# zju3dv/pvnet

Measured on NVIDIA H100. Metric: images/sec (480x640, K=9) backbone+vote, higher is better.
Workload: dtype tf32 (fp32 storage, fp32 accumulate; vote fp32/fp64)

## Files before the change

### include/pvnet_b200.h

```cpp
#ifndef PVNET_B200_H_
#define PVNET_B200_H_

#include <stddef.h>
#include <stdint.h>

#ifdef __cplusplus
extern "C" {
#endif

#if defined(__GNUC__)
#define PVNET_API __attribute__((visibility("default")))
#else
#define PVNET_API
#endif

typedef void *pvnet_stream_t;

enum {
    PVNET_OK = 0,
    PVNET_E_INVALID = -1,
    PVNET_E_WORKSPACE = -2,
    PVNET_E_CUDA = -3,
    PVNET_E_STATE = -4
};
// ... 171 lines not shown
    int32_t *counts;
    double *sil_obj;
    int32_t *pair_idx;
    double *normal_eq;
} pvnet_refine_trace_t;
PVNET_API int pvnet_refine_workspace_bytes(int b, int h, int w, int max_points, size_t *bytes);
PVNET_API int pvnet_refine_poses(const uint8_t *mask, const double *poses_in, const float *K, int k_per_image,
                                 const float *verts, const int32_t *faces, int nv, int nf, int b, int h, int w,
                                 float near_clip, float far_clip, int rounds, float gate, int max_points,
                                 double *poses_out, int32_t *info, double *dist, const pvnet_refine_trace_t *trace,
                                 void *workspace, size_t workspace_bytes, pvnet_stream_t stream);

PVNET_API int pvnet_refine_poses_keypoints(const uint8_t *mask, const double *poses_in, const float *K, int k_per_image,
                                           const float *verts, const int32_t *faces, int nv, int nf, int b, int h,
                                           int w, float near_clip, float far_clip, int rounds, float gate,
                                           int max_points, const float *keypoints, const float *points_3d,
                                           const float *weights_2d, int nk, double keypoint_weight, double *poses_out,
                                           int32_t *info, double *dist, double *cost,
                                           const pvnet_refine_trace_t *trace, double *keypoint_eq, void *workspace,
                                           size_t workspace_bytes, pvnet_stream_t stream);

typedef struct {
    int32_t *pair_idx;
    int32_t *counts;
    double *X;
    double *Y;
    double *n;
    double *normal_eq;
} pvnet_refine_depth_trace_t;
PVNET_API int pvnet_refine_depth_workspace_bytes(int b, int h, int w, int max_points, size_t *bytes);
PVNET_API int pvnet_refine_poses_depth(const uint8_t *mask, const void *depth, int depth_is_u16, float depth_scale,
                                       const double *poses_in, const float *K, int k_per_image, const float *verts,
                                       const int32_t *faces, int nv, int nf, int b, int h, int w, float near_clip,
                                       float far_clip, int rounds, double gate, int max_points, double *poses_out,
                                       int32_t *info, double *dist, const pvnet_refine_depth_trace_t *trace,
                                       void *workspace, size_t workspace_bytes, pvnet_stream_t stream);

PVNET_API int pvnet_generate_hypothesis_vanishing_point(const float *direct, const float *coords, const int32_t *idxs,
                                                        float *hypo, int tn, int vn, int hn, pvnet_stream_t stream);
PVNET_API int pvnet_voting_for_hypothesis_vanishing_point(const float *direct, const float *coords, const float *hypo,
                                                          uint8_t *inliers, int32_t *counts, int tn, int vn, int hn,
                                                          float inlier_thresh, pvnet_stream_t stream);

PVNET_API long long pvnet_launch_count(void);
PVNET_API void pvnet_launch_count_reset(void);


PVNET_API int pvnet_conv2d_nhwc(const float *in, int in_cs, int in_co, int Cin,
                                const float *w_packed, const float *bias,
                                const float *res, int res_cs, int res_co,
                                float *out, int out_cs, int out_co, int Cout,
                                int b, int H, int W, int ksize, int stride, int dilation,
                                int act, int round_out, pvnet_stream_t stream);

PVNET_API int pvnet_conv2d_nhwc_wgrad_workspace_bytes(int Cin, int Cout, int b, int H, int W, int ksize,
                                                      size_t *bytes);
PVNET_API int pvnet_conv2d_nhwc_wgrad(const float *in, int in_cs, int in_co, int Cin,
                                      const float *dout, int dout_cs, int dout_co, int Cout, float *dw,
                                      int b, int H, int W, int ksize, int dilation,
                                      void *workspace, size_t workspace_bytes, pvnet_stream_t stream);
PVNET_API int pvnet_zero_insert2x_nhwc(const float *in, int in_cs, int in_co, int C, float *out, int out_cs,
                                       int out_co, int b, int H, int W, pvnet_stream_t stream);

PVNET_API int pvnet_upsample2x_nhwc(const float *in, int C, float *out, int out_cs, int out_co, int b, int h, int w,
                                    pvnet_stream_t stream);
PVNET_API int pvnet_upsample2x_backward_nhwc(const float *dout, int dout_cs, int dout_co, int C, float *din, int b,
                                             int h, int w, pvnet_stream_t stream);

typedef struct pvnet_batchnorm {
    const float *weight;
    const float *bias;
    float *running_mean;
    float *running_var;
    int batch_stats;
    double factor;
    double eps;
    double *saved;
    float *coef;
} pvnet_batchnorm_t;
PVNET_API int pvnet_batchnorm_workspace_bytes(int form, int C, long long npix, size_t *bytes);
PVNET_API int pvnet_batchnorm_act_forward(int form, int act, const float *x, const float *z, long long npix, int C,
                                          const pvnet_batchnorm_t *bn, const pvnet_batchnorm_t *bn_z, float *y,
                                          void *workspace, size_t workspace_bytes, pvnet_stream_t stream);
PVNET_API int pvnet_batchnorm_act_backward(int form, int act, const float *dy, const float *x, const float *z,
                                           long long npix, int C, const pvnet_batchnorm_t *bn,
                                           const pvnet_batchnorm_t *bn_z, float *dx, float *dz, float *dweight,
                                           float *dbias, float *dweight_z, float *dbias_z, void *workspace,
                                           size_t workspace_bytes, pvnet_stream_t stream);

PVNET_API int pvnet_stem_s2d_nhwc(const void *image, int image_is_u8, const float *mean3, const float *std3,
                                  const float *w_s2d, const float *bias, float *s2d, float *out, float *img, int img_cs,
                                  int img_co, int b, int H, int W, pvnet_stream_t stream);
PVNET_API int pvnet_stem_s2d_half_nhwc(const void *image, int image_is_u8, const float *mean3, const float *std3,
                                       const float *w_s2d, const float *bias, float *s2d, float *out, float *img,
                                       int img_cs, int img_co, int b, int H, int W, pvnet_stream_t stream);
PVNET_API int pvnet_stem_s2d_wgrad_workspace_bytes(int b, int H, int W, size_t *bytes);
PVNET_API int pvnet_stem_s2d_wgrad(const float *s2d, const float *dout, float *dw, int b, int H, int W,
                                   void *workspace, size_t workspace_bytes, pvnet_stream_t stream);
PVNET_API int pvnet_maxpool3x3s2_nhwc(const float *in, float *out, uint8_t *code, int b, int H, int W, int C,
                                      pvnet_stream_t stream);
PVNET_API int pvnet_maxpool3x3s2_backward_nhwc(const float *dout, const uint8_t *code, float *din, int b, int H, int W,
                                               int C, pvnet_stream_t stream);
PVNET_API int pvnet_head1x1_nchw(const float *y, const float *w, const float *bias, float *out, int b, int H, int W,
                                 int Cin, int Cout, pvnet_stream_t stream);
PVNET_API int pvnet_head1x1_backward_workspace_bytes(int b, int H, int W, int Cin, int Cout, size_t *bytes);
PVNET_API int pvnet_head1x1_backward(const float *dout, const float *y, const float *w, float *dy, float *dw,
// ... 67 lines not shown
```

### pvnet_b200/_native.py

```python
from __future__ import annotations

import ctypes
import os
import threading

_HERE = os.path.dirname(os.path.abspath(__file__))
LIB_PATH = os.path.join(_HERE, "_lib", "libpvnet_b200.so")

_lock = threading.Lock()
_lib = None

c_void_p = ctypes.c_void_p
c_int = ctypes.c_int
c_float = ctypes.c_float
c_size_t = ctypes.c_size_t
c_int64_p = ctypes.POINTER(ctypes.c_int64)


class BatchNormParams(ctypes.Structure):
    _fields_ = [("weight", c_void_p), ("bias", c_void_p), ("running_mean", c_void_p), ("running_var", c_void_p),
                ("batch_stats", c_int), ("factor", ctypes.c_double), ("eps", ctypes.c_double),
                ("saved", c_void_p), ("coef", c_void_p)]


# ... 97 lines not shown
    "pvnet_refine_depth_workspace_bytes": (c_int, [c_int, c_int, c_int, c_int, ctypes.POINTER(c_size_t)]),
    "pvnet_refine_poses_depth": (c_int, [c_void_p, c_void_p, c_int, c_float, c_void_p, c_void_p, c_int, c_void_p,
                                         c_void_p, c_int, c_int, c_int, c_int, c_int, c_float, c_float, c_int,
                                         ctypes.c_double, c_int, c_void_p, c_void_p, c_void_p,
                                         ctypes.POINTER(RefineDepthTrace), c_void_p, c_size_t, c_void_p]),
    "pvnet_generate_hypothesis":(c_int, [c_void_p, c_void_p, c_void_p, c_void_p, c_int, c_int, c_int, c_void_p]),
    "pvnet_voting_for_hypothesis": (c_int, [c_void_p, c_void_p, c_void_p, c_void_p, c_int, c_int, c_int, c_float,
                                            c_void_p]),
    "pvnet_generate_hypothesis_vanishing_point": (c_int, [c_void_p, c_void_p, c_void_p, c_void_p, c_int, c_int, c_int,
                                                          c_void_p]),
    "pvnet_voting_for_hypothesis_vanishing_point": (c_int, [c_void_p, c_void_p, c_void_p, c_void_p, c_void_p, c_int, c_int,
                                                            c_int, c_float, c_void_p]),
    "pvnet_vote_counts": (c_int, [c_void_p, c_void_p, c_void_p, c_void_p, c_int, c_int, c_int, c_float, c_void_p]),
    "pvnet_conv2d_nhwc": (c_int, [c_void_p, c_int, c_int, c_int, c_void_p, c_void_p, c_void_p, c_int, c_int,
                                  c_void_p, c_int, c_int, c_int, c_int, c_int, c_int, c_int, c_int, c_int,
                                  c_int, c_int, c_void_p]),
    "pvnet_conv2d_nhwc_wgrad_workspace_bytes": (c_int, [c_int, c_int, c_int, c_int, c_int, c_int,
                                                        ctypes.POINTER(c_size_t)]),
    "pvnet_conv2d_nhwc_wgrad": (c_int, [c_void_p, c_int, c_int, c_int, c_void_p, c_int, c_int, c_int, c_void_p,
                                        c_int, c_int, c_int, c_int, c_int, c_void_p, c_size_t, c_void_p]),
    "pvnet_zero_insert2x_nhwc": (c_int, [c_void_p, c_int, c_int, c_int, c_void_p, c_int, c_int, c_int, c_int, c_int,
                                         c_void_p]),
    "pvnet_upsample2x_nhwc": (c_int, [c_void_p, c_int, c_void_p, c_int, c_int, c_int, c_int, c_int, c_void_p]),
    "pvnet_upsample2x_backward_nhwc": (c_int, [c_void_p, c_int, c_int, c_int, c_void_p, c_int, c_int, c_int, c_void_p]),
    "pvnet_batchnorm_workspace_bytes": (c_int, [c_int, c_int, ctypes.c_longlong, ctypes.POINTER(c_size_t)]),
    "pvnet_batchnorm_act_forward": (c_int, [c_int, c_int, c_void_p, c_void_p, ctypes.c_longlong, c_int, c_bn_p, c_bn_p,
                                            c_void_p, c_void_p, c_size_t, c_void_p]),
    "pvnet_batchnorm_act_backward": (c_int, [c_int, c_int, c_void_p, c_void_p, c_void_p, ctypes.c_longlong, c_int,
                                             c_bn_p, c_bn_p, c_void_p, c_void_p, c_void_p, c_void_p, c_void_p, c_void_p,
                                             c_void_p, c_size_t, c_void_p]),
    "pvnet_stem_s2d_nhwc": (c_int, [c_void_p, c_int, ctypes.POINTER(c_float), ctypes.POINTER(c_float), c_void_p,
                                    c_void_p, c_void_p, c_void_p, c_void_p, c_int, c_int, c_int, c_int, c_int,
                                    c_void_p]),
    "pvnet_stem_s2d_half_nhwc": (c_int, [c_void_p, c_int, ctypes.POINTER(c_float), ctypes.POINTER(c_float), c_void_p,
                                         c_void_p, c_void_p, c_void_p, c_void_p, c_int, c_int, c_int, c_int, c_int,
                                         c_void_p]),
    "pvnet_stem_s2d_wgrad_workspace_bytes": (c_int, [c_int, c_int, c_int, ctypes.POINTER(c_size_t)]),
    "pvnet_stem_s2d_wgrad": (c_int, [c_void_p, c_void_p, c_void_p, c_int, c_int, c_int, c_void_p, c_size_t, c_void_p]),
    "pvnet_maxpool3x3s2_nhwc": (c_int, [c_void_p, c_void_p, c_void_p, c_int, c_int, c_int, c_int, c_void_p]),
    "pvnet_maxpool3x3s2_backward_nhwc": (c_int, [c_void_p, c_void_p, c_void_p, c_int, c_int, c_int, c_int, c_void_p]),
    "pvnet_head1x1_nchw": (c_int, [c_void_p, c_void_p, c_void_p, c_void_p, c_int, c_int, c_int, c_int, c_int,
                                   c_void_p]),
    "pvnet_head1x1_backward_workspace_bytes": (c_int, [c_int, c_int, c_int, c_int, c_int, ctypes.POINTER(c_size_t)]),
    "pvnet_head1x1_backward": (c_int, [c_void_p, c_void_p, c_void_p, c_void_p, c_void_p, c_void_p, c_int, c_int,
                                       c_int, c_int, c_int, c_void_p, c_size_t, c_void_p]),
    "pvnet_head3x3_nchw": (c_int, [c_void_p, c_void_p, c_void_p, c_void_p, c_int, c_int, c_int, c_int, c_void_p]),
    "pvnet_head3x3_backward_workspace_bytes": (c_int, [c_int, c_int, c_int, c_int, ctypes.POINTER(c_size_t)]),
    "pvnet_head3x3_backward": (c_int, [c_void_p, c_void_p, c_void_p, c_void_p, c_void_p, c_void_p, c_int, c_int,
                                       c_int, c_int, c_void_p, c_size_t, c_void_p]),
    "pvnet_adam_step": (c_int, [ctypes.POINTER(AdamTensor), c_int, ctypes.c_double, ctypes.c_double, ctypes.c_double,
                                ctypes.c_double, ctypes.c_double, ctypes.c_int64, c_void_p]),
    "pvnet_adam_chunk_tensors": (c_int, []),
    "pvnet_conv_set_mode": (c_int, [c_int]),
    "pvnet_backbone_create": (c_int, [c_int, c_int, c_int, c_int, c_int, c_int, c_int, ctypes.POINTER(c_void_p)]),
    "pvnet_backbone_create_trunk": (c_int, [c_int, ctypes.POINTER(c_int), c_int, c_int, c_int, c_int, c_int, c_int,
                                            c_int, ctypes.POINTER(c_void_p)]),
    "pvnet_backbone_create_trunk_2o": (c_int, [c_int, ctypes.POINTER(c_int), c_int, c_int, c_int, c_int, c_int,
                                               c_int, ctypes.POINTER(c_void_p)]),
    "pvnet_backbone_create_detector": (c_int, [c_int, ctypes.POINTER(c_int), c_int, ctypes.POINTER(c_void_p)]),
    "pvnet_backbone_output_scale": (c_int, [c_void_p]),
    "pvnet_backbone_destroy": (None, [c_void_p]),
    "pvnet_backbone_num_convs": (c_int, []),
    "pvnet_backbone_handle_num_convs": (c_int, [c_void_p]),
    "pvnet_backbone_set_conv": (c_int, [c_void_p, c_int, c_void_p, c_void_p]),
    "pvnet_backbone_set_output_layout": (c_int, [c_void_p, c_int]),
    "pvnet_backbone_workspace_bytes": (c_int, [c_void_p, c_int, c_int, c_int, ctypes.POINTER(c_size_t)]),
    "pvnet_backbone_forward": (c_int, [c_void_p, c_void_p, c_int, c_int, c_int, c_void_p, c_void_p, c_int,
                                       c_void_p, c_size_t, c_void_p]),
    "pvnet_backbone_forward_u8": (c_int, [c_void_p, c_void_p, ctypes.POINTER(c_float), ctypes.POINTER(c_float), c_int, c_int,
                                          c_int, c_void_p, c_void_p, c_int, c_void_p, c_size_t, c_void_p]),
    "pvnet_jpeg_available": (c_int, []),
    "pvnet_jpeg_decoder_create": (c_int, [ctypes.POINTER(c_void_p)]),
    "pvnet_jpeg_decoder_destroy": (None, [c_void_p]),
    "pvnet_jpeg_decode_batch": (c_int, [c_void_p, ctypes.POINTER(ctypes.c_char_p), ctypes.POINTER(c_size_t), c_int, c_int,
                                        c_int, c_void_p, c_void_p]),
    "pvnet_backbone_num_stages": (c_int, []),
    "pvnet_backbone_stage_name": (ctypes.c_char_p, [c_int]),
    "pvnet_backbone_handle_num_stages": (c_int, [c_void_p]),
    "pvnet_backbone_handle_stage_name": (ctypes.c_char_p, [c_void_p, c_int]),
    "pvnet_backbone_run_stage": (c_int, [c_void_p, c_int, c_void_p, c_int, c_int, c_int, c_void_p, c_void_p, c_int,
                                         c_void_p, c_size_t, c_void_p]),
}


def lib():
    global _lib
    if _lib is None:
        with _lock:
            if _lib is None:
                if not os.path.exists(LIB_PATH):
                    raise RuntimeError(
                        f"{LIB_PATH} is missing: build it with `python -m pvnet_b200._build` "
                        "(or __graft_entry__.build()).  pvnet_b200 has no CPU or PyTorch fallback.")
                L = ctypes.CDLL(LIB_PATH)
                for name, (res, args) in SIGNATURES.items():
                    fn = getattr(L, name)
                    fn.restype = res
                    fn.argtypes = args
                _lib = L
    return _lib


def check(status: int, what: str):
    if status != 0:
        msg = lib().pvnet_last_error()
        raise RuntimeError(f"{what} failed (status {status}): {msg.decode() if msg else '?'}")
# ... 9 lines not shown
```

### pvnet_b200/conv.py

```python
from __future__ import annotations

import ctypes

import torch
from torch.autograd.function import once_differentiable

from . import _native

ACT_NONE, ACT_RELU, ACT_LEAKY = 0, 1, 2
MODE_AUTO, MODE_PER_TAP, MODE_COLUMN = 0, 1, 2


def set_mode(mode: int):
    _native.check(_native.lib().pvnet_conv_set_mode(int(mode)), "pvnet_conv_set_mode")


def round_tf32(t: torch.Tensor) -> torch.Tensor:
    i = t.contiguous().view(torch.int32)
    i = (i + 0x1000) & ~0x1FFF
    return i.view(torch.float32)


def fold_bn(weight, bn_weight=None, bn_bias=None, bn_mean=None, bn_var=None, eps=1e-5, conv_bias=None):
    w = weight.detach().to(torch.float64)
    cout = w.shape[0]
    b = torch.zeros(cout, dtype=torch.float64, device=w.device) if conv_bias is None else conv_bias.detach().double()
    if bn_weight is not None:
        scale = bn_weight.detach().double() / torch.sqrt(bn_var.detach().double() + eps)
        w = w * scale[:, None, None, None]
        b = (b - bn_mean.detach().double()) * scale + bn_bias.detach().double()
    return w.float(), b.float()


def cin_padded(cin: int) -> int:
    return 16 if cin == 16 else (cin + 31) // 32 * 32


def pack_weight(w: torch.Tensor, cin_pad: int | None = None, cout_pad: int | None = None, tf32: bool = True):
    cout, cin, kh, kw = w.shape
    cin_pad = cin_padded(cin) if cin_pad is None else cin_pad
    cout_pad = cout if cout_pad is None else cout_pad
    p = torch.zeros(cout_pad, kh * kw, cin_pad, dtype=torch.float32, device=w.device)
    p[:cout, :, :cin] = w.permute(0, 2, 3, 1).reshape(cout, kh * kw, cin)
    return round_tf32(p) if tf32 else p.contiguous()


def pack_stem_s2d(w: torch.Tensor) -> torch.Tensor:
    cout = w.shape[0]
    out = torch.zeros(cout, 4, 4, 16, dtype=torch.float32, device=w.device)
    for ty in range(4):
        for py in range(2):
            kh = 2 * ty + py - 1
            if not 0 <= kh <= 6:
                continue
            for tx in range(4):
                for px in range(2):
                    kw = 2 * tx + px - 1
                    if not 0 <= kw <= 6:
                        continue
                    ch = (py * 2 + px) * 3
                    out[:, ty, tx, ch:ch + 3] = w[:, :, kh, kw]
    return round_tf32(out)


def _p(t):
    return None if t is None else ctypes.c_void_p(t.data_ptr())

# ... 596 lines not shown
```

### pvnet_b200/csrc/conv_tc.cu

```cuda
#include "conv_tc.cuh"
#include "ptx.cuh"

#include <cstdlib>
#include <mutex>
#include <new>

namespace pvnet {

struct ConvGeom {
    int Ho, Wo;
    int tiles_x, tiles_y, total_m_tiles;
    int TH, TW;
    int taps, cin_chunks, cin_pad;
    int Cout, BN;
    int out_cs, out_co;
    int res_cs, res_co;
    int act;
    int round_out;
    signed char tap_map[9];
    short tap_ox[9], tap_oy[9];
    int n_items;
    int stages;
};

struct AMaps {
    CUtensorMap m[4];
};

constexpr int CONV_THREADS = 288;
constexpr int CONV_KC = 32;
constexpr int CONV_A_BYTES = 128 * CONV_KC * 4;
constexpr int CONV_SLAB = 32;
constexpr int CONV_SLAB_BYTES = 128 * CONV_SLAB * 4;
constexpr int CONV_EPI_BAR = 1;

template <int BN>
__global__ void __launch_bounds__(CONV_THREADS, 1)
    k_conv_tap(const __grid_constant__ AMaps amaps, const __grid_constant__ CUtensorMap tmB,
               const __grid_constant__ CUtensorMap tmOut, const __grid_constant__ CUtensorMap tmRes,
               const __grid_constant__ ConvGeom g, const float *__restrict__ bias, const int has_res)
{
    constexpr int B_BYTES = BN * CONV_KC * 4;
    constexpr int STAGE_BYTES = CONV_A_BYTES + B_BYTES;
    constexpr int SLABS = BN / CONV_SLAB;
    const int STAGES = g.stages;
    extern __shared__ uint8_t smem_raw[];
    uint8_t *smem = reinterpret_cast<uint8_t *>((reinterpret_cast<uintptr_t>(smem_raw) + 1023) & ~uintptr_t(1023));
    uint8_t *slab = smem + (size_t)STAGES * STAGE_BYTES;
    uint64_t *full = reinterpret_cast<uint64_t *>(slab + 2 * CONV_SLAB_BYTES);
    uint64_t *empty = full + STAGES;
    uint64_t *res_full = empty + STAGES;
    uint64_t *res_free = res_full + 2;

    const int warp = threadIdx.x >> 5, lane = threadIdx.x & 31;
    const int tiles_per_img = g.tiles_x * g.tiles_y;
    const int n_tiles_n = g.Cout / BN;
    const int nkb = g.taps * g.cin_chunks;
    const int unit = (int)blockIdx.x, nunits = (int)gridDim.x;
    auto item_tile = [&](int item, int &m_tile, int &n0) {
        m_tile = item / n_tiles_n;
        n0 = (item - m_tile * n_tiles_n) * BN;
    };

    if (threadIdx.x == 0) {
        for (int s = 0; s < STAGES; ++s) {
            ptx::mbar_init(&full[s], 1);
            ptx::mbar_init(&empty[s], 8);
        }
        for (int i = 0; i < 2; ++i) {
            ptx::mbar_init(&res_full[i], 1);
            ptx::mbar_init(&res_free[i], 1);
        }
        ptx::fence_barrier_init();
    }
    __syncthreads();

    if (warp == 8) {
        if (lane == 0) {
            int r_item = has_res ? unit : g.n_items, r_slab = 0;
            uint32_t rq = 0;
            auto poll_res = [&]() {
                if (r_item >= g.n_items) return;
                const uint32_t b = rq & 1u;
                if (!ptx::mbar_test_wait(&res_free[b], ((rq >> 1) & 1u) ^ 1u)) return;
                int m_tile, n0;
                item_tile(r_item, m_tile, n0);
                const int img = m_tile / tiles_per_img;
                const int trem = m_tile - img * tiles_per_img;
                const int tyi = trem / g.tiles_x, txi = trem - tyi * g.tiles_x;
                ptx::mbar_arrive_expect_tx(&res_full[b], (uint32_t)CONV_SLAB_BYTES);
                ptx::tma_load_4d(slab + b * CONV_SLAB_BYTES, &tmRes, &res_full[b], n0 + r_slab * CONV_SLAB, txi * g.TW,
                                 tyi * g.TH, img);
                ++rq;
                if (++r_slab == SLABS) {
                    r_slab = 0;
                    r_item += nunits;
                }
            };
            int s = 0;
            uint32_t ph = 0;
            for (int item = unit; item < g.n_items; item += nunits) {
                int m_tile, n0;
                item_tile(item, m_tile, n0);
                const int img = m_tile / tiles_per_img;
                const int trem = m_tile - img * tiles_per_img;
                const int tyi = trem / g.tiles_x, txi = trem - tyi * g.tiles_x;
                const int y0 = tyi * g.TH, x0 = txi * g.TW;
                for (int tap = 0; tap < g.taps; ++tap)
                    for (int cc = 0; cc < g.cin_chunks; ++cc) {
                        poll_res();
                        while (!(has_res ? ptx::mbar_test_wait(&empty[s], ph ^ 1u) : ptx::mbar_try_wait(&empty[s], ph ^ 1u)))
                            poll_res();
                        ptx::mbar_arrive_expect_tx(&full[s], (uint32_t)STAGE_BYTES);
                        uint8_t *sa = smem + (size_t)s * STAGE_BYTES;
                        ptx::tma_load_4d(sa, &amaps.m[g.tap_map[tap]], &full[s], cc * CONV_KC, x0 + g.tap_ox[tap],
                                         y0 + g.tap_oy[tap], img);
                        ptx::tma_load_2d(sa + CONV_A_BYTES, &tmB, &full[s], tap * g.cin_pad + cc * CONV_KC, n0);
                        if (++s == STAGES) {
                            s = 0;
                            ph ^= 1u;
                        }
                    }
            }
            while (r_item < g.n_items) poll_res();
        }
    } else {
        const int wg = warp >> 2, wq = warp & 3;
        const int g8 = lane >> 2, t4 = lane & 3;
        const uint32_t smem_u = ptx::smem_u32(smem);
        int s = 0;
        uint32_t ph = 0, sq = 0;
        for (int item = unit; item < g.n_items; item += nunits) {
            float acc[BN / 2];
#pragma unroll
            for (int i = 0; i < BN / 2; ++i) acc[i] = 0.f;
            int prev = -1;
            for (int kb = 0; kb < nkb; ++kb) {
                ptx::mbar_wait(&full[s], ph);
                const uint32_t sa = smem_u + (uint32_t)s * (uint32_t)STAGE_BYTES;
                const uint64_t adesc = ptx::make_kmajor_desc(sa + (uint32_t)(wg * 64 * 128), 128);
                const uint64_t bdesc = ptx::make_kmajor_desc(sa + (uint32_t)CONV_A_BYTES, 128);
                ptx::wgmma_fence();
#pragma unroll
                for (int k = 0; k < CONV_KC / 8; ++k)
                    ptx::Wgmma<BN>::ss(acc, adesc + (uint64_t)(2 * k), bdesc + (uint64_t)(2 * k), (kb | k) != 0 ? 1u : 0u);
                ptx::wgmma_commit();
                ptx::wgmma_wait<1>();
                ptx::fence_regs(acc);
                if (prev >= 0 && lane == 0) ptx::mbar_arrive(&empty[prev]);
                prev = s;
                if (++s == STAGES) {
                    s = 0;
                    ph ^= 1u;
                }
            }
            ptx::wgmma_wait<0>();
            ptx::fence_regs(acc);
            if (lane == 0) ptx::mbar_arrive(&empty[prev]);

            int m_tile, n0;
            item_tile(item, m_tile, n0);
            const int img = m_tile / tiles_per_img;
            const int trem = m_tile - img * tiles_per_img;
            const int tyi = trem / g.tiles_x, txi = trem - tyi * g.tiles_x;
            const uint32_t row_off = (uint32_t)((wg * 64 + wq * 16 + g8) * 128 + (t4 & 1) * 8);
            const uint32_t swz = (uint32_t)(((t4 >> 1) ^ g8) << 4);
            const uint32_t slab_u = ptx::smem_u32(slab);
#pragma unroll
            for (int j = 0; j < SLABS; ++j, ++sq) {
                const uint32_t b = sq & 1u;
                const uint32_t base = slab_u + b * (uint32_t)CONV_SLAB_BYTES + row_off;
                float2 bv[4];
#pragma unroll
                for (int jj = 0; jj < 4; ++jj)
                    bv[jj] = __ldg(reinterpret_cast<const float2 *>(bias + n0 + CONV_SLAB * j + 8 * jj + 2 * t4));
                if (has_res) ptx::mbar_wait(&res_full[b], (sq >> 1) & 1u);
                else ptx::named_bar_sync(CONV_EPI_BAR, 256);
#pragma unroll
                for (int jj = 0; jj < 4; ++jj)
#pragma unroll
                    for (int h = 0; h < 2; ++h) {
                        const uint32_t addr = base + (uint32_t)(h * 8 * 128) + (swz ^ (uint32_t)(32 * jj));
                        const int a = 4 * (4 * j + jj) + 2 * h;
                        float2 v = make_float2(acc[a] + bv[jj].x, acc[a + 1] + bv[jj].y);
                        if (has_res) {
                            const float2 r = ptx::lds64(addr);
                            v.x += r.x;
                            v.y += r.y;
                        }
                        v.x = epi_act(v.x, g.act, g.round_out);
                        v.y = epi_act(v.y, g.act, g.round_out);
                        ptx::sts64(addr, v);
                    }
                ptx::fence_proxy_async();
                ptx::named_bar_sync(CONV_EPI_BAR, 256);
                if (threadIdx.x == 0) {
                    ptx::tma_store_4d(&tmOut, slab + b * CONV_SLAB_BYTES, n0 + CONV_SLAB * j, txi * g.TW, tyi * g.TH, img);
                    ptx::tma_store_commit();
                    if (j == SLABS - 1) ptx::tma_store_wait_read();
                    else ptx::tma_store_wait_read1();
                    if (has_res) {
                        if (j > 0) ptx::mbar_arrive(&res_free[b ^ 1u]);
                        if (j == SLABS - 1) ptx::mbar_arrive(&res_free[b]);
                    }
                }
                __syncwarp();
            }
        }
        if (threadIdx.x == 0) ptx::tma_store_wait_all();
    }
}

typedef CUresult (*EncodeTiledFn)(CUtensorMap *, CUtensorMapDataType, cuuint32_t, void *, const cuuint64_t *,
                                  const cuuint64_t *, const cuuint32_t *, const cuuint32_t *, CUtensorMapInterleave,
                                  CUtensorMapSwizzle, CUtensorMapL2promotion, CUtensorMapFloatOOBfill);

static EncodeTiledFn encode_fn()
{
    static EncodeTiledFn fn = nullptr;
    static std::once_flag once;
    std::call_once(once, [] {
        void *p = nullptr;
        cudaDriverEntryPointQueryResult q;
        if (cudaGetDriverEntryPoint("cuTensorMapEncodeTiled", &p, cudaEnableDefault, &q) == cudaSuccess &&
            q == cudaDriverEntryPointSuccess)
            fn = reinterpret_cast<EncodeTiledFn>(p);
    });
    return fn;
}

int tma_encode(CUtensorMap *m, const void *base, int rank, const cuuint64_t *dims, const cuuint64_t *strides_bytes,
               const cuuint32_t *box, int swizzle_bytes)
{
    EncodeTiledFn fn = encode_fn();
    if (!fn) {
        set_error("cuTensorMapEncodeTiled entry point unavailable");
        return PVNET_E_CUDA;
    }
    cuuint32_t estr[5] = {1, 1, 1, 1, 1};
    const CUtensorMapSwizzle sw = swizzle_bytes == 128 ? CU_TENSOR_MAP_SWIZZLE_128B
                                  : swizzle_bytes == 64 ? CU_TENSOR_MAP_SWIZZLE_64B
                                                        : CU_TENSOR_MAP_SWIZZLE_32B;
    CUresult r = fn(m, CU_TENSOR_MAP_DATA_TYPE_FLOAT32, (cuuint32_t)rank, const_cast<void *>(base), dims,
                    strides_bytes, box, estr, CU_TENSOR_MAP_INTERLEAVE_NONE, sw, CU_TENSOR_MAP_L2_PROMOTION_L2_128B,
                    CU_TENSOR_MAP_FLOAT_OOB_FILL_NONE);
    if (r == CUDA_ERROR_INVALID_CONTEXT || r == CUDA_ERROR_NOT_INITIALIZED) {
        cudaFree(nullptr);
        r = fn(m, CU_TENSOR_MAP_DATA_TYPE_FLOAT32, (cuuint32_t)rank, const_cast<void *>(base), dims, strides_bytes, box, estr,
               CU_TENSOR_MAP_INTERLEAVE_NONE, sw, CU_TENSOR_MAP_L2_PROMOTION_L2_128B, CU_TENSOR_MAP_FLOAT_OOB_FILL_NONE);
    }
    if (r != CUDA_SUCCESS) {
        set_error("cuTensorMapEncodeTiled failed with CUresult %d (rank %d, dims %llu %llu, box %u %u, swizzle %d)",
                  (int)r, rank, (unsigned long long)dims[0], (unsigned long long)dims[1], box[0], box[1],
                  swizzle_bytes);
        return PVNET_E_CUDA;
    }
    return PVNET_OK;
}

struct ConvPlan {
    AMaps amaps;
    CUtensorMap tmB;
    CUtensorMap tmOut, tmRes;
    ConvGeom g;
    dim3 grid;
    size_t smem;
    const float *bias;
    int has_res;
};

int conv_plan(const ConvDesc &d, ConvPlan *p)
{
    PV_CHECK_ARG(d.in && d.w && d.bias && d.out, "conv: null pointer");
    PV_CHECK_ARG(!d.in2, "conv: a second input source is only supported by the column kernel");
    PV_CHECK_ARG(d.ksize == 1 || d.ksize == 3, "conv: kernel size %d unsupported", d.ksize);
    PV_CHECK_ARG(d.stride == 1 || d.stride == 2, "conv: stride %d unsupported", d.stride);
    PV_CHECK_ARG(d.stride == 1 || (d.dilation == 1 && d.H % 2 == 0 && d.W % 2 == 0),
                 "conv: stride 2 needs dilation 1 and even H,W");
    PV_CHECK_ARG(d.Cout % 32 == 0, "conv: Cout %d must be a multiple of 32", d.Cout);
    PV_CHECK_ARG(d.in_cs % 4 == 0 && d.in_co % 4 == 0 && d.out_cs % 4 == 0 && d.out_co % 4 == 0,
                 "conv: channel strides/offsets must be multiples of 4 floats");
    PV_CHECK_ARG(!d.res || (d.res_cs % 4 == 0 && d.res_co % 4 == 0), "conv: residual stride/offset alignment");
    PV_CHECK_ARG(((uintptr_t)d.in % 16 == 0) && ((uintptr_t)d.w % 16 == 0) && ((uintptr_t)d.out % 16 == 0) &&
                     ((uintptr_t)d.bias % 16 == 0),
                 "conv: pointers must be 16-byte aligned");
    PV_CHECK_ARG(d.Cin % 4 == 0, "conv: Cin %d must be a multiple of 4", d.Cin);
    const int kc = CONV_KC;
    ConvGeom &g = p->g;
    g.Ho = d.H / d.stride;
    g.Wo = d.W / d.stride;
    g.TH = 8;
    g.TW = 16;
    g.tiles_x = (g.Wo + g.TW - 1) / g.TW;
    g.tiles_y = (g.Ho + g.TH - 1) / g.TH;
    g.total_m_tiles = g.tiles_x * g.tiles_y * d.b;
    g.taps = d.ksize * d.ksize;
    g.cin_chunks = (d.Cin + kc - 1) / kc;
    g.cin_pad = g.cin_chunks * kc;
    g.Cout = d.Cout;
    {
        const long long sms = sm_count() > 0 ? sm_count() : 1;
        long long best = -1;
        for (int bn = 256; bn >= 32; bn >>= 1) {
            if (d.Cout % bn) continue;
            const long long items = (long long)g.total_m_tiles * (d.Cout / bn);
            const long long cost = (items + sms - 1) / sms * (CONV_A_BYTES + bn * kc * 4);
            if (best < 0 || cost < best) {
                best = cost;
                g.BN = bn;
            }
        }
    }
    g.out_cs = d.out_cs;
    g.out_co = d.out_co;
    g.res_cs = d.res_cs;
    g.res_co = d.res_co;
    g.act = d.act;
    g.round_out = d.round_out;
    const int pad = d.dilation * (d.ksize - 1) / 2;
    for (int t = 0; t < g.taps; ++t) {
        const int kh = t / d.ksize, kw = t - kh * d.ksize;
        if (d.stride == 1) {
            g.tap_map[t] = 0;
            g.tap_ox[t] = (short)(kw * d.dilation - pad);
            g.tap_oy[t] = (short)(kh * d.dilation - pad);
        } else {
            const int dy = kh - pad, dx = kw - pad;
            const int py = dy & 1, px = dx & 1;
            g.tap_map[t] = (signed char)(py * 2 + px);
            g.tap_oy[t] = (short)((dy - py) / 2);
            g.tap_ox[t] = (short)((dx - px) / 2);
        }
    }
    const int swz = kc * 4;
    const int nplanes = d.stride == 2 ? 4 : 1;
    for (int pl = 0; pl < nplanes; ++pl) {
        const int py = pl >> 1, px = pl & 1;
        const float *base = d.in + d.in_co + ((size_t)py * d.W + px) * d.in_cs;
        cuuint64_t dims[4] = {(cuuint64_t)d.Cin, (cuuint64_t)(d.W / d.stride), (cuuint64_t)(d.H / d.stride),
                              (cuuint64_t)d.b};
        cuuint64_t strides[3] = {(cuuint64_t)d.stride * d.in_cs * 4, (cuuint64_t)d.stride * d.W * d.in_cs * 4,
                                 (cuuint64_t)d.H * d.W * d.in_cs * 4};
        cuuint32_t box[4] = {(cuuint32_t)kc, (cuuint32_t)g.TW, (cuuint32_t)g.TH, 1};
        int rc = tma_encode(&p->amaps.m[pl], base, 4, dims, strides, box, swz);
        if (rc) return rc;
    }
    for (int pl = nplanes; pl < 4; ++pl) p->amaps.m[pl] = p->amaps.m[0];
    {
        cuuint64_t dims[2] = {(cuuint64_t)g.taps * g.cin_pad, (cuuint64_t)d.Cout};
        cuuint64_t strides[1] = {(cuuint64_t)g.taps * g.cin_pad * 4};
        cuuint32_t box[2] = {(cuuint32_t)kc, (cuuint32_t)g.BN};
        int rc = tma_encode(&p->tmB, d.w, 2, dims, strides, box, swz);
        if (rc) return rc;
    }
    {
        cuuint64_t dims[4] = {(cuuint64_t)d.Cout, (cuuint64_t)g.Wo, (cuuint64_t)g.Ho, (cuuint64_t)d.b};
        cuuint32_t box[4] = {(cuuint32_t)CONV_SLAB, (cuuint32_t)g.TW, (cuuint32_t)g.TH, 1};
        cuuint64_t ostr[3] = {(cuuint64_t)d.out_cs * 4, (cuuint64_t)g.Wo * d.out_cs * 4,
                              (cuuint64_t)g.Ho * g.Wo * d.out_cs * 4};
        int rc = tma_encode(&p->tmOut, d.out + d.out_co, 4, dims, ostr, box, CONV_SLAB * 4);
        if (rc) return rc;
        p->tmRes = p->tmOut;
        if (d.res) {
            PV_CHECK_ARG((uintptr_t)d.res % 16 == 0, "conv: pointers must be 16-byte aligned");
            cuuint64_t rstr[3] = {(cuuint64_t)d.res_cs * 4, (cuuint64_t)g.Wo * d.res_cs * 4,
                                  (cuuint64_t)g.Ho * g.Wo * d.res_cs * 4};
            rc = tma_encode(&p->tmRes, d.res + d.res_co, 4, dims, rstr, box, CONV_SLAB * 4);
            if (rc) return rc;
        }
    }
    const size_t stage_b = (size_t)CONV_A_BYTES + (size_t)g.BN * kc * 4;
    int st = (int)((227 * 1024 - 1024 - 256 - 2 * CONV_SLAB_BYTES) / stage_b);
    if (st > 8) st = 8;
    g.stages = st;
    p->smem = 1024 + (size_t)st * stage_b + 2 * CONV_SLAB_BYTES + 256;
    g.n_items = g.total_m_tiles * (d.Cout / g.BN);
    long long grid = (long long)sm_count();
    if (grid > g.n_items) grid = g.n_items;
    p->grid = dim3((unsigned)grid);
    p->bias = d.bias;
    p->has_res = d.res != nullptr;
    return PVNET_OK;
}

template <int BN>
int conv_launch_t(const ConvPlan &p, cudaStream_t s)
{
    const cudaError_t attr_err = ensure_max_smem((const void *)k_conv_tap<BN>, 227 * 1024);
    PV_CUDA(attr_err);
    k_conv_tap<BN><<<p.grid, CONV_THREADS, p.smem, s>>>(p.amaps, p.tmB, p.tmOut, p.tmRes, p.g, p.bias, p.has_res);
    PV_LAUNCHED("k_conv_tap");
    return PVNET_OK;
}

int conv_launch(const ConvPlan &p, cudaStream_t s)
{
    if (p.g.BN == 256) return conv_launch_t<256>(p, s);
    if (p.g.BN == 128) return conv_launch_t<128>(p, s);
    if (p.g.BN == 64) return conv_launch_t<64>(p, s);
    return conv_launch_t<32>(p, s);
}

size_t conv_plan_size() { return sizeof(ConvPlan); }
int conv_plan_at(const ConvDesc &d, void *storage) { return conv_plan(d, new (storage) ConvPlan()); }
int conv_launch_at(const void *storage, cudaStream_t s) { return conv_launch(*static_cast<const ConvPlan *>(storage), s); }

}

extern "C" {

int pvnet_conv2d_nhwc(const float *in, int in_cs, int in_co, int Cin, const float *w_packed, const float *bias,
                      const float *res, int res_cs, int res_co, float *out, int out_cs, int out_co, int Cout, int b,
                      int H, int W, int ksize, int stride, int dilation, int act, int round_out,
                      pvnet_stream_t stream)
{
    pvnet::ConvDesc d{in, in_cs, in_co, Cin, w_packed, bias, res, res_cs, res_co, out, out_cs, out_co, Cout,
                      b, H, W, ksize, stride, dilation, act, round_out};
    const bool col = pvnet::g_conv_mode == 2 || (pvnet::g_conv_mode == 0 && pvnet::conv_col_eligible(d));
    if (col) {
        alignas(64) unsigned char storage[2048];
        static_assert(sizeof(storage) >= 1024, "plan storage");
        if (pvnet::conv_col_plan_size() > sizeof(storage)) {
            pvnet::set_error("column plan larger than its stack storage");
            return PVNET_E_STATE;
        }
        int rc = pvnet::conv_col_plan_at(d, nullptr, storage);
        if (rc) return rc;
        return pvnet::conv_col_launch_at(storage, (cudaStream_t)stream);
    }
    pvnet::ConvPlan plan;
    int rc = pvnet::conv_plan(d, &plan);
    if (rc) return rc;
    return pvnet::conv_launch(plan, (cudaStream_t)stream);
}

}
```

Before: 1720.

## Add cost-model tile scheduler with tail-split launches and multi-image tiles

Replaces the simple BN choice in the tap conv with a cost model that estimates k-block clocks per BN and decides whether to split the work into two launches: a main launch with full waves and a tail launch with a smaller BN that fits in one wave. It also considers a 4x16x2-image tile geometry that changes how many M tiles there are and how they quantize against the SM count. The goal is to cut wave-quantization idle time on the last partial wave of the persistent grid. In exchange it adds an extra launch, and its heuristic constants (feed rate, launch overhead) could choose a worse schedule for some layers. A debug API that exposes the schedule is also added.

```diff
diff --git a/include/pvnet_b200.h b/include/pvnet_b200.h
--- a/include/pvnet_b200.h
+++ b/include/pvnet_b200.h
@@ -247,6 +247,9 @@
                                 float *out, int out_cs, int out_co, int Cout,
                                 int b, int H, int W, int ksize, int stride, int dilation,
                                 int act, int round_out, pvnet_stream_t stream);
+
+PVNET_API int pvnet_conv_tap_schedule(int b, int H, int W, int Cin, int Cout, int ksize, int stride, int sms,
+                                      int *out, int out_len);
 
 PVNET_API int pvnet_conv2d_nhwc_wgrad_workspace_bytes(int Cin, int Cout, int b, int H, int W, int ksize,
                                                       size_t *bytes);
diff --git a/pvnet_b200/_native.py b/pvnet_b200/_native.py
--- a/pvnet_b200/_native.py
+++ b/pvnet_b200/_native.py
@@ -173,6 +173,7 @@
                                 ctypes.c_double, ctypes.c_double, ctypes.c_int64, c_void_p]),
     "pvnet_adam_chunk_tensors": (c_int, []),
     "pvnet_conv_set_mode": (c_int, [c_int]),
+    "pvnet_conv_tap_schedule": (c_int, [c_int, c_int, c_int, c_int, c_int, c_int, c_int, c_int, c_void_p, c_int]),
     "pvnet_backbone_create": (c_int, [c_int, c_int, c_int, c_int, c_int, c_int, c_int, ctypes.POINTER(c_void_p)]),
     "pvnet_backbone_create_trunk": (c_int, [c_int, ctypes.POINTER(c_int), c_int, c_int, c_int, c_int, c_int, c_int,
                                             c_int, ctypes.POINTER(c_void_p)]),
diff --git a/pvnet_b200/conv.py b/pvnet_b200/conv.py
--- a/pvnet_b200/conv.py
+++ b/pvnet_b200/conv.py
@@ -13,6 +13,15 @@
 
 def set_mode(mode: int):
     _native.check(_native.lib().pvnet_conv_set_mode(int(mode)), "pvnet_conv_set_mode")
+
+
+def tap_schedule(b: int, H: int, W: int, cin: int, cout: int, ksize: int, stride: int = 1, sms: int = 132) -> dict:
+    out = (ctypes.c_int * 17)()
+    _native.check(_native.lib().pvnet_conv_tap_schedule(int(b), int(H), int(W), int(cin), int(cout), int(ksize),
+                                                        int(stride), int(sms), out, 17), "pvnet_conv_tap_schedule")
+    v = list(out)
+    launches = [dict(zip(("bn", "m0", "m_tiles", "items", "grid"), v[7 + 5 * i:12 + 5 * i])) for i in range(v[6])]
+    return dict(zip(("th", "tw", "ti", "tiles_x", "tiles_y", "m_tiles"), v[:6]), launches=launches)
 
 
 def round_tf32(t: torch.Tensor) -> torch.Tensor:
diff --git a/pvnet_b200/csrc/conv_tc.cu b/pvnet_b200/csrc/conv_tc.cu
--- a/pvnet_b200/csrc/conv_tc.cu
+++ b/pvnet_b200/csrc/conv_tc.cu
@@ -10,7 +10,8 @@
 struct ConvGeom {
     int Ho, Wo;
     int tiles_x, tiles_y, total_m_tiles;
-    int TH, TW;
+    int TH, TW, TI;
+    int m0;
     int taps, cin_chunks, cin_pad;
     int Cout, BN;
     int out_cs, out_co;
@@ -53,13 +54,22 @@
     uint64_t *res_free = res_full + 2;
 
     const int warp = threadIdx.x >> 5, lane = threadIdx.x & 31;
-    const int tiles_per_img = g.tiles_x * g.tiles_y;
+    const int tiles_per_grp = g.tiles_x * g.tiles_y;
     const int n_tiles_n = g.Cout / BN;
     const int nkb = g.taps * g.cin_chunks;
     const int unit = (int)blockIdx.x, nunits = (int)gridDim.x;
     auto item_tile = [&](int item, int &m_tile, int &n0) {
-        m_tile = item / n_tiles_n;
-        n0 = (item - m_tile * n_tiles_n) * BN;
+        const int mi = item / n_tiles_n;
+        m_tile = g.m0 + mi;
+        n0 = (item - mi * n_tiles_n) * BN;
+    };
+    auto tile_origin = [&](int m_tile, int &x0, int &y0, int &img) {
+        const int grp = m_tile / tiles_per_grp;
+        const int trem = m_tile - grp * tiles_per_grp;
+        const int tyi = trem / g.tiles_x;
+        x0 = (trem - tyi * g.tiles_x) * g.TW;
+        y0 = tyi * g.TH;
+        img = grp * g.TI;
     };
 
     if (threadIdx.x == 0) {
@@ -83,14 +93,11 @@
                 if (r_item >= g.n_items) return;
                 const uint32_t b = rq & 1u;
                 if (!ptx::mbar_test_wait(&res_free[b], ((rq >> 1) & 1u) ^ 1u)) return;
-                int m_tile, n0;
+                int m_tile, n0, x0, y0, img;
                 item_tile(r_item, m_tile, n0);
-                const int img = m_tile / tiles_per_img;
-                const int trem = m_tile - img * tiles_per_img;
-                const int tyi = trem / g.tiles_x, txi = trem - tyi * g.tiles_x;
+                tile_origin(m_tile, x0, y0, img);
                 ptx::mbar_arrive_expect_tx(&res_full[b], (uint32_t)CONV_SLAB_BYTES);
-                ptx::tma_load_4d(slab + b * CONV_SLAB_BYTES, &tmRes, &res_full[b], n0 + r_slab * CONV_SLAB, txi * g.TW,
-                                 tyi * g.TH, img);
+                ptx::tma_load_4d(slab + b * CONV_SLAB_BYTES, &tmRes, &res_full[b], n0 + r_slab * CONV_SLAB, x0, y0, img);
                 ++rq;
                 if (++r_slab == SLABS) {
                     r_slab = 0;
@@ -100,12 +107,9 @@
             int s = 0;
             uint32_t ph = 0;
             for (int item = unit; item < g.n_items; item += nunits) {
-                int m_tile, n0;
+                int m_tile, n0, x0, y0, img;
                 item_tile(item, m_tile, n0);
-                const int img = m_tile / tiles_per_img;
-                const int trem = m_tile - img * tiles_per_img;
-                const int tyi = trem / g.tiles_x, txi = trem - tyi * g.tiles_x;
-                const int y0 = tyi * g.TH, x0 = txi * g.TW;
+                tile_origin(m_tile, x0, y0, img);
                 for (int tap = 0; tap < g.taps; ++tap)
                     for (int cc = 0; cc < g.cin_chunks; ++cc) {
                         poll_res();
@@ -158,11 +162,9 @@
             ptx::fence_regs(acc);
             if (lane == 0) ptx::mbar_arrive(&empty[prev]);
 
-            int m_tile, n0;
+            int m_tile, n0, x0, y0, img;
             item_tile(item, m_tile, n0);
-            const int img = m_tile / tiles_per_img;
-            const int trem = m_tile - img * tiles_per_img;
-            const int tyi = trem / g.tiles_x, txi = trem - tyi * g.tiles_x;
+            tile_origin(m_tile, x0, y0, img);
             const uint32_t row_off = (uint32_t)((wg * 64 + wq * 16 + g8) * 128 + (t4 & 1) * 8);
             const uint32_t swz = (uint32_t)(((t4 >> 1) ^ g8) << 4);
             const uint32_t slab_u = ptx::smem_u32(slab);
@@ -195,7 +197,7 @@
                 ptx::fence_proxy_async();
                 ptx::named_bar_sync(CONV_EPI_BAR, 256);
                 if (threadIdx.x == 0) {
-                    ptx::tma_store_4d(&tmOut, slab + b * CONV_SLAB_BYTES, n0 + CONV_SLAB * j, txi * g.TW, tyi * g.TH, img);
+                    ptx::tma_store_4d(&tmOut, slab + b * CONV_SLAB_BYTES, n0 + CONV_SLAB * j, x0, y0, img);
                     ptx::tma_store_commit();
                     if (j == SLABS - 1) ptx::tma_store_wait_read();
                     else ptx::tma_store_wait_read1();
@@ -258,13 +260,91 @@
     return PVNET_OK;
 }
 
+struct TapLaunch {
+    int bn;
+    int m0, m_tiles;
+    int n_items, grid;
+};
+struct TapSchedule {
+    int TH, TW, TI, tiles_x, tiles_y, total_m_tiles;
+    int nlaunch;
+    TapLaunch l[2];
+};
+
+constexpr long long TAP_RHO = 36;
+constexpr long long TAP_LAUNCH_CLOCKS = 8000;
+
+static long long tap_kblock_clocks(int bn)
+{
+    const long long mma = 1024LL * bn / 256;
+    const long long feed = ((long long)CONV_A_BYTES + (long long)bn * CONV_KC * 4 + TAP_RHO - 1) / TAP_RHO;
+    return mma > feed ? mma : feed;
+}
+
+static long long tap_launches(int Cout, int nkb, int sms, TapSchedule *t)
+{
+    const long long M = t->total_m_tiles, S = sms > 0 ? sms : 1;
+    auto rounds = [&](long long items) { return (items + S - 1) / S; };
+    long long best = -1;
+    for (int bn = 256; bn >= 32; bn >>= 1) {
+        if (Cout % bn) continue;
+        const long long nn = Cout / bn;
+        const long long one = rounds(M * nn) * nkb * tap_kblock_clocks(bn);
+        if (best < 0 || one < best) {
+            best = one;
+            t->nlaunch = 1;
+            t->l[0] = {bn, 0, (int)M, 0, 0};
+        }
+        const long long mm = (M * nn / S) * S / nn;
+        if (mm == 0 || mm == M) continue;
+        int bt = 0;
+        for (int c = 32; c < bn && !bt; c <<= 1)
+            if (Cout % c == 0 && (M - mm) * (Cout / c) <= S) bt = c;
+        if (!bt) continue;
+        const long long two =
+            rounds(mm * nn) * nkb * tap_kblock_clocks(bn) + nkb * tap_kblock_clocks(bt) + TAP_LAUNCH_CLOCKS;
+        if (two < best) {
+            best = two;
+            t->nlaunch = 2;
+            t->l[0] = {bn, 0, (int)mm, 0, 0};
+            t->l[1] = {bt, (int)mm, (int)(M - mm), 0, 0};
+        }
+    }
+    for (int i = 0; i < t->nlaunch; ++i) {
+        TapLaunch &l = t->l[i];
+        l.n_items = l.m_tiles * (Cout / l.bn);
+        l.grid = (int)(S < l.n_items ? S : l.n_items);
+    }
+    return best;
+}
+
+static void tap_schedule(int b, int Ho, int Wo, int Cout, int nkb, int sms, TapSchedule *t)
+{
+    auto geometry = [&](TapSchedule *u, int th, int ti) {
+        u->TW = 16;
+        u->TH = th;
+        u->TI = ti;
+        u->tiles_x = (Wo + u->TW - 1) / u->TW;
+        u->tiles_y = (Ho + u->TH - 1) / u->TH;
+        u->total_m_tiles = u->tiles_x * u->tiles_y * (b / u->TI);
+    };
+    geometry(t, 8, 1);
+    const long long cost = tap_launches(Cout, nkb, sms, t);
+    if (b % 2 == 0 && Ho % 4 == 0 && Wo % 16 == 0) {
+        TapSchedule u{};
+        geometry(&u, 4, 2);
+        if (tap_launches(Cout, nkb, sms, &u) < cost) *t = u;
+    }
+}
+
 struct ConvPlan {
     AMaps amaps;
-    CUtensorMap tmB;
     CUtensorMap tmOut, tmRes;
-    ConvGeom g;
-    dim3 grid;
-    size_t smem;
+    CUtensorMap tmB[2];
+    ConvGeom g[2];
+    dim3 grid[2];
+    size_t smem[2];
+    int nlaunch;
     const float *bias;
     int has_res;
 };
@@ -286,31 +366,21 @@
                  "conv: pointers must be 16-byte aligned");
     PV_CHECK_ARG(d.Cin % 4 == 0, "conv: Cin %d must be a multiple of 4", d.Cin);
     const int kc = CONV_KC;
-    ConvGeom &g = p->g;
+    ConvGeom g{};
     g.Ho = d.H / d.stride;
     g.Wo = d.W / d.stride;
-    g.TH = 8;
-    g.TW = 16;
-    g.tiles_x = (g.Wo + g.TW - 1) / g.TW;
-    g.tiles_y = (g.Ho + g.TH - 1) / g.TH;
-    g.total_m_tiles = g.tiles_x * g.tiles_y * d.b;
     g.taps = d.ksize * d.ksize;
     g.cin_chunks = (d.Cin + kc - 1) / kc;
     g.cin_pad = g.cin_chunks * kc;
+    TapSchedule t;
+    tap_schedule(d.b, g.Ho, g.Wo, d.Cout, g.taps * g.cin_chunks, sm_count(), &t);
+    g.TH = t.TH;
+    g.TW = t.TW;
+    g.TI = t.TI;
+    g.tiles_x = t.tiles_x;
+    g.tiles_y = t.tiles_y;
+    g.total_m_tiles = t.total_m_tiles;
     g.Cout = d.Cout;
-    {
-        const long long sms = sm_count() > 0 ? sm_count() : 1;
-        long long best = -1;
-        for (int bn = 256; bn >= 32; bn >>= 1) {
-            if (d.Cout % bn) continue;
-            const long long items = (long long)g.total_m_tiles * (d.Cout / bn);
-            const long long cost = (items + sms - 1) / sms * (CONV_A_BYTES + bn * kc * 4);
-            if (best < 0 || cost < best) {
-                best = cost;
-                g.BN = bn;
-            }
-        }
-    }
     g.out_cs = d.out_cs;
     g.out_co = d.out_co;
     g.res_cs = d.res_cs;
@@ -318,18 +388,18 @@
     g.act = d.act;
     g.round_out = d.round_out;
     const int pad = d.dilation * (d.ksize - 1) / 2;
-    for (int t = 0; t < g.taps; ++t) {
-        const int kh = t / d.ksize, kw = t - kh * d.ksize;
+    for (int tp = 0; tp < g.taps; ++tp) {
+        const int kh = tp / d.ksize, kw = tp - kh * d.ksize;
         if (d.stride == 1) {
-            g.tap_map[t] = 0;
-            g.tap_ox[t] = (short)(kw * d.dilation - pad);
-            g.tap_oy[t] = (short)(kh * d.dilation - pad);
+            g.tap_map[tp] = 0;
+            g.tap_ox[tp] = (short)(kw * d.dilation - pad);
+            g.tap_oy[tp] = (short)(kh * d.dilation - pad);
         } else {
             const int dy = kh - pad, dx = kw - pad;
             const int py = dy & 1, px = dx & 1;
-            g.tap_map[t] = (signed char)(py * 2 + px);
-            g.tap_oy[t] = (short)((dy - py) / 2);
-            g.tap_ox[t] = (short)((dx - px) / 2);
+            g.tap_map[tp] = (signed char)(py * 2 + px);
+            g.tap_oy[tp] = (short)((dy - py) / 2);
+            g.tap_ox[tp] = (short)((dx - px) / 2);
         }
     }
     const int swz = kc * 4;
@@ -341,21 +411,14 @@
                               (cuuint64_t)d.b};
         cuuint64_t strides[3] = {(cuuint64_t)d.stride * d.in_cs * 4, (cuuint64_t)d.stride * d.W * d.in_cs * 4,
                                  (cuuint64_t)d.H * d.W * d.in_cs * 4};
-        cuuint32_t box[4] = {(cuuint32_t)kc, (cuuint32_t)g.TW, (cuuint32_t)g.TH, 1};
+        cuuint32_t box[4] = {(cuuint32_t)kc, (cuuint32_t)g.TW, (cuuint32_t)g.TH, (cuuint32_t)g.TI};
         int rc = tma_encode(&p->amaps.m[pl], base, 4, dims, strides, box, swz);
         if (rc) return rc;
     }
     for (int pl = nplanes; pl < 4; ++pl) p->amaps.m[pl] = p->amaps.m[0];
     {
-        cuuint64_t dims[2] = {(cuuint64_t)g.taps * g.cin_pad, (cuuint64_t)d.Cout};
-        cuuint64_t strides[1] = {(cuuint64_t)g.taps * g.cin_pad * 4};
-        cuuint32_t box[2] = {(cuuint32_t)kc, (cuuint32_t)g.BN};
-        int rc = tma_encode(&p->tmB, d.w, 2, dims, strides, box, swz);
-        if (rc) return rc;
-    }
-    {
         cuuint64_t dims[4] = {(cuuint64_t)d.Cout, (cuuint64_t)g.Wo, (cuuint64_t)g.Ho, (cuuint64_t)d.b};
-        cuuint32_t box[4] = {(cuuint32_t)CONV_SLAB, (cuuint32_t)g.TW, (cuuint32_t)g.TH, 1};
+        cuuint32_t box[4] = {(cuuint32_t)CONV_SLAB, (cuuint32_t)g.TW, (cuuint32_t)g.TH, (cuuint32_t)g.TI};
         cuuint64_t ostr[3] = {(cuuint64_t)d.out_cs * 4, (cuuint64_t)g.Wo * d.out_cs * 4,
                               (cuuint64_t)g.Ho * g.Wo * d.out_cs * 4};
         int rc = tma_encode(&p->tmOut, d.out + d.out_co, 4, dims, ostr, box, CONV_SLAB * 4);
@@ -369,36 +432,53 @@
             if (rc) return rc;
         }
     }
-    const size_t stage_b = (size_t)CONV_A_BYTES + (size_t)g.BN * kc * 4;
-    int st = (int)((227 * 1024 - 1024 - 256 - 2 * CONV_SLAB_BYTES) / stage_b);
-    if (st > 8) st = 8;
-    g.stages = st;
-    p->smem = 1024 + (size_t)st * stage_b + 2 * CONV_SLAB_BYTES + 256;
-    g.n_items = g.total_m_tiles * (d.Cout / g.BN);
-    long long grid = (long long)sm_count();
-    if (grid > g.n_items) grid = g.n_items;
-    p->grid = dim3((unsigned)grid);
+    p->nlaunch = t.nlaunch;
+    for (int i = 0; i < t.nlaunch; ++i) {
+        const TapLaunch &l = t.l[i];
+        ConvGeom &gi = p->g[i];
+        gi = g;
+        gi.BN = l.bn;
+        gi.m0 = l.m0;
+        gi.n_items = l.n_items;
+        cuuint64_t dims[2] = {(cuuint64_t)g.taps * g.cin_pad, (cuuint64_t)d.Cout};
+        cuuint64_t strides[1] = {(cuuint64_t)g.taps * g.cin_pad * 4};
+        cuuint32_t box[2] = {(cuuint32_t)kc, (cuuint32_t)l.bn};
+        int rc = tma_encode(&p->tmB[i], d.w, 2, dims, strides, box, swz);
+        if (rc) return rc;
+        const size_t stage_b = (size_t)CONV_A_BYTES + (size_t)l.bn * kc * 4;
+        int st = (int)((227 * 1024 - 1024 - 256 - 2 * CONV_SLAB_BYTES) / stage_b);
+        if (st > 8) st = 8;
+        gi.stages = st;
+        p->smem[i] = 1024 + (size_t)st * stage_b + 2 * CONV_SLAB_BYTES + 256;
+        p->grid[i] = dim3((unsigned)l.grid);
+    }
     p->bias = d.bias;
     p->has_res = d.res != nullptr;
     return PVNET_OK;
 }
 
 template <int BN>
-int conv_launch_t(const ConvPlan &p, cudaStream_t s)
+int conv_launch_t(const ConvPlan &p, int i, cudaStream_t s)
 {
     const cudaError_t attr_err = ensure_max_smem((const void *)k_conv_tap<BN>, 227 * 1024);
     PV_CUDA(attr_err);
-    k_conv_tap<BN><<<p.grid, CONV_THREADS, p.smem, s>>>(p.amaps, p.tmB, p.tmOut, p.tmRes, p.g, p.bias, p.has_res);
+    k_conv_tap<BN><<<p.grid[i], CONV_THREADS, p.smem[i], s>>>(p.amaps, p.tmB[i], p.tmOut, p.tmRes, p.g[i], p.bias,
+                                                              p.has_res);
     PV_LAUNCHED("k_conv_tap");
     return PVNET_OK;
 }
 
 int conv_launch(const ConvPlan &p, cudaStream_t s)
 {
-    if (p.g.BN == 256) return conv_launch_t<256>(p, s);
-    if (p.g.BN == 128) return conv_launch_t<128>(p, s);
-    if (p.g.BN == 64) return conv_launch_t<64>(p, s);
-    return conv_launch_t<32>(p, s);
+    for (int i = 0; i < p.nlaunch; ++i) {
+        const int bn = p.g[i].BN;
+        const int rc = bn == 256 ? conv_launch_t<256>(p, i, s)
+                       : bn == 128 ? conv_launch_t<128>(p, i, s)
+                       : bn == 64  ? conv_launch_t<64>(p, i, s)
+                                   : conv_launch_t<32>(p, i, s);
+        if (rc) return rc;
+    }
+    return PVNET_OK;
 }
 
 size_t conv_plan_size() { return sizeof(ConvPlan); }
@@ -434,4 +514,26 @@
     return pvnet::conv_launch(plan, (cudaStream_t)stream);
 }
 
-}
+int pvnet_conv_tap_schedule(int b, int H, int W, int Cin, int Cout, int ksize, int stride, int sms, int *out,
+                            int out_len)
+{
+    PV_CHECK_ARG(out && out_len >= 17, "conv schedule: out needs 17 ints");
+    PV_CHECK_ARG(b >= 1 && H >= 1 && W >= 1 && Cin >= 1 && sms >= 1, "conv schedule: dimension out of range");
+    PV_CHECK_ARG(Cout >= 32 && Cout % 32 == 0, "conv schedule: Cout %d must be a multiple of 32", Cout);
+    PV_CHECK_ARG(ksize == 1 || ksize == 3, "conv schedule: kernel size %d unsupported", ksize);
+    PV_CHECK_ARG(stride == 1 || (stride == 2 && H % 2 == 0 && W % 2 == 0), "conv schedule: stride %d unsupported",
+                 stride);
+    pvnet::TapSchedule t{};
+    pvnet::tap_schedule(b, H / stride, W / stride, Cout, ksize * ksize * ((Cin + 31) / 32), sms, &t);
+    const int head[7] = {t.TH, t.TW, t.TI, t.tiles_x, t.tiles_y, t.total_m_tiles, t.nlaunch};
+    for (int i = 0; i < 17; ++i) out[i] = 0;
+    for (int i = 0; i < 7; ++i) out[i] = head[i];
+    for (int i = 0; i < t.nlaunch; ++i) {
+        const pvnet::TapLaunch &l = t.l[i];
+        const int v[5] = {l.bn, l.m0, l.m_tiles, l.n_items, l.grid};
+        for (int j = 0; j < 5; ++j) out[7 + 5 * i + j] = v[j];
+    }
+    return PVNET_OK;
+}
+
+}
```

After: 1751 (median of 6 runs). +1.8%, better.
